# Ze-Yang/Context-Transformer

Hardware: AMD Instinct MI355X
Metric: images/sec fwd+NMS (higher is better)
Workload: dtype f32

## Files before the change

### context-transformer_amd/csrc/ct_conv.hip

```cpp
#include "ct_common.h"
#include "ct_conv_emit.h"
#include "ct_conv_launch.h"
#include "ct_device.h"
#include "ct_f16x2.h"
#include <algorithm>
#include <cmath>
#include <type_traits>
#include <cstdlib>

namespace {

using ctdet::f32x16;
using ctdet::i32x4;
using ctdet::kInvalidOff;
using ctdet::kMaxBufBytes;
using ctdet::make_rsrc;


struct ConvArgs {
    const float* in;
    const float* wpk;
    const float* scale;
    const float* shift;
    const float* res;
    const float* lo;
    float* out;
    unsigned in_bytes, w_bytes;
    int Cin, H, W, in_ctot, in_coff;
    int M, M_pad, nsteps;
    int stride, pad_h, pad_w, dil;
    int OW, OHW, Npix;
    int out_ctot, out_coff, res_ctot, res_coff;
    float res_scale;
    int relu;
    int nseg;
    ct_out_segment seg[3];
    int tiles_m, tiles_n;
    int transposed;
    int ksplit, steps_per_split;
    float* ws;
    unsigned* out_amax;
};

template <int KH, int KW, int CPB, int BM, int BN, int WAVES_M, int MINW>
__global__ __launch_bounds__(256, MINW) void conv_igemm_f32(const ConvArgs a)
{
    constexpr int KHW = KH * KW;
    constexpr int BK = CPB * KHW;
    constexpr int WAVES_N = 4 / WAVES_M;
    constexpr int WM = BM / WAVES_M, WN = BN / WAVES_N;
    constexpr int TM = WM / 32, TN = WN / 32;
    constexpr int RPP = 256 / BN;
    constexpr int NB = BK / RPP;
    constexpr int A_F4 = BK * BM / 4;
    constexpr int NA = (A_F4 + 255) / 256;
    static_assert(BK % 2 == 0 && BK % RPP == 0, "k-step must be even and divide into passes");
    static_assert(TM >= 1 && TN >= 1 && BN >= 64, "wave tile");

    extern __shared__ __attribute__((aligned(16))) float smem[];
    float* const As = smem;
    float* const Bs = smem + 2 * BK * BM;

    const int tid = threadIdx.x;
    const int lane = tid & 63;
    const int l31 = lane & 31;
    const int hsel = lane >> 5;
    const int wave = __builtin_amdgcn_readfirstlane(tid >> 6);
    const int wm0 = (wave % WAVES_M) * WM;
    const int wn0 = (wave / WAVES_M) * WN;

    int wg;
    {
        const int nwg = a.tiles_m * a.tiles_n;
        const int bid = blockIdx.x;
        const int xcd = bid & 7, local = bid >> 3;
        const int q = nwg >> 3, r = nwg & 7;
        wg = (xcd < r ? xcd * (q + 1) : r * (q + 1) + (xcd - r) * q) + local;
    }
    const int m0 = (wg % a.tiles_m) * BM;
    const int n0 = (wg / a.tiles_m) * BN;

    const __amdgpu_buffer_rsrc_t rin = make_rsrc(a.in, a.in_bytes);
    const __amdgpu_buffer_rsrc_t rw = make_rsrc(a.wpk, a.w_bytes);

    const int bp = tid % BN;
    const int rowgrp = __builtin_amdgcn_readfirstlane(tid / BN);
    const int HW = a.H * a.W;
    int img_base, oh_, ow_;
    bool pvalid;
    {
        const int P = n0 + bp;
        pvalid = P < a.Npix;
        const int Pc = pvalid ? P : 0;
        const int n = Pc / a.OHW;
        const int s = Pc - n * a.OHW;
        oh_ = s / a.OW;
        ow_ = s - oh_ * a.OW;
        img_base = (n * a.in_ctot + a.in_coff) * HW;
    }
    auto tap_offset = [&](int kh, int kw) -> int {
        int ih, iw;
        bool ok = pvalid;
        if (!a.transposed) {
            ih = oh_ * a.stride - a.pad_h + kh * a.dil;
            iw = ow_ * a.stride - a.pad_w + kw * a.dil;
        } else {
            const int th = oh_ + a.pad_h - kh * a.dil, tw = ow_ + a.pad_w - kw * a.dil;
            ih = th / a.stride;
            iw = tw / a.stride;
            ok = ok && th >= 0 && tw >= 0 && ih * a.stride == th && iw * a.stride == tw;
        }
        ok = ok && (unsigned)ih < (unsigned)a.H && (unsigned)iw < (unsigned)a.W;
        return ok ? img_base + ih * a.W + iw : -1;
    };

    int a_voff[NA];
    int a_lds[NA];
#pragma unroll
    for (int j = 0; j < NA; ++j) {
        int f = tid + 256 * j;
        if (f >= A_F4) f %= A_F4;
        const int arow = f / (BM / 4), ac4 = f % (BM / 4);
        const int col = m0 + ac4 * 4;
        a_voff[j] = (col < a.M_pad) ? (arow * a.M_pad + col) * 4 : kInvalidOff;
        a_lds[j] = arow * BM + ac4 * 4;
    }
    const int a_step_bytes = BK * a.M_pad * 4;

    int b_voff[NB];
    int b_chan[NB];
#pragma unroll
    for (int i = 0; i < NB; ++i) {
        const int r = rowgrp + RPP * i;
        const int c = r / KHW, tap = r - c * KHW;
        const int kh = tap / KW, kw = tap - kh * KW;
        const int off = tap_offset(kh, kw);
        b_voff[i] = off >= 0 ? off * 4 : kInvalidOff;
        b_chan[i] = c;
    }
    const int chan_bytes = HW * 4;

    i32x4 areg[NA];
    float breg[NB];

    auto load_elem = [&](int e, int step) {
        if (e < NA) {
            areg[e] = __builtin_amdgcn_raw_buffer_load_b128(rw, a_voff[e], step * a_step_bytes, 0);
        } else {
            const int i = e - NA;
            const int ci = step * CPB + b_chan[i];
            const int soff = (ci < a.Cin ? ci : 0) * chan_bytes;
            breg[i] = __builtin_bit_cast(float, __builtin_amdgcn_raw_buffer_load_b32(rin, b_voff[i], soff, 0));
        }
    };
    auto store_elem = [&](int e, int buf) {
        if (e < NA) {
            *reinterpret_cast<i32x4*>(As + buf * (BK * BM) + a_lds[e]) = areg[e];
        } else {
            const int i = e - NA;
            Bs[buf * (BK * BN) + (rowgrp + RPP * i) * BN + bp] = breg[i];
        }
    };
    auto load_tile = [&](int step) {
#pragma unroll
        for (int e = 0; e < NA + NB; ++e) load_elem(e, step);
    };
    auto store_tile = [&](int buf) {
#pragma unroll
        for (int e = 0; e < NA + NB; ++e) store_elem(e, buf);
    };

    f32x16 acc[TM][TN];
#pragma unroll
    for (int i = 0; i < TM; ++i)
#pragma unroll
        for (int j = 0; j < TN; ++j)
#pragma unroll
            for (int r = 0; r < 16; ++r) acc[i][j][r] = 0.f;

    constexpr int NKP = BK / 2;
    constexpr int NST = NA + NB;
    constexpr int NSLOT = NKP - 1;
    constexpr int WPS = (NST + NSLOT - 1) / NSLOT;

    const int s0 = blockIdx.y * a.steps_per_split;
    const int s1 = min(a.nsteps, s0 + a.steps_per_split);
    auto k_step = [&](int step, auto store_c, auto load_c) {
        constexpr bool STORE = decltype(store_c)::value, LOAD = decltype(load_c)::value;
        const int buf = (step - s0) & 1;
        const float* Ab = As + buf * (BK * BM) + hsel * BM + wm0 + l31;
        const float* Bb = Bs + buf * (BK * BN) + hsel * BN + wn0 + l31;
        float av[2][TM], bv[2][TN];
#pragma unroll
        for (int i = 0; i < TM; ++i) av[0][i] = Ab[i * 32];
#pragma unroll
        for (int j = 0; j < TN; ++j) bv[0][j] = Bb[j * 32];
#pragma unroll
        for (int kp = 0; kp < NKP; ++kp) {
            const int cur = kp & 1;
            if (kp + 1 < NKP) {
#pragma unroll
                for (int i = 0; i < TM; ++i) av[cur ^ 1][i] = Ab[(2 * kp + 2) * BM + i * 32];
#pragma unroll
                for (int j = 0; j < TN; ++j) bv[cur ^ 1][j] = Bb[(2 * kp + 2) * BN + j * 32];
            }
#pragma unroll
            for (int q = 0; q < WPS; ++q) {
                const int e = kp * WPS + q;
                if (e < NST) {
                    if (STORE) store_elem(e, buf ^ 1);
                    if (LOAD) load_elem(e, step + 2);
                }
            }
#pragma unroll
            for (int i = 0; i < TM; ++i)
#pragma unroll
                for (int j = 0; j < TN; ++j)
                    acc[i][j] = __builtin_amdgcn_mfma_f32_32x32x2f32(av[cur][i], bv[cur][j], acc[i][j], 0, 0, 0);
            __builtin_amdgcn_sched_barrier(0);
        }
        __syncthreads();
    };
    using T_ = std::true_type;
    using F_ = std::false_type;

    load_tile(s0);
    store_tile(0);
    if (s1 - s0 > 1) load_tile(s0 + 1);
    __syncthreads();
    int step = s0;
    for (; step + 2 < s1; ++step) k_step(step, T_{}, T_{});
    if (step + 1 < s1) { k_step(step, T_{}, F_{}); ++step; }
    k_step(step, F_{}, F_{});

    if (a.ksplit > 1) {
        float* const slab = a.ws + (size_t)blockIdx.y * a.M * a.Npix;
#pragma unroll
        for (int j = 0; j < TN; ++j) {
            const int P = n0 + wn0 + j * 32 + l31;
            if (P >= a.Npix) continue;
#pragma unroll
            for (int i = 0; i < TM; ++i)
#pragma unroll
                for (int r = 0; r < 16; ++r) {
                    const int co = m0 + wm0 + i * 32 + (r & 3) + 8 * (r >> 2) + 4 * hsel;
                    if (co < a.M) slab[(size_t)co * a.Npix + P] = acc[i][j][r];
                }
        }
        return;
    }

    float* const ev = smem;
    for (int i = tid; i < BM; i += 256) ctdet::stage_epilogue_vector<BM>(ev, a, m0, i);
    __syncthreads();
    const bool track = a.out_amax != nullptr;
#pragma unroll
    for (int j = 0; j < TN; ++j) {
        const int P = n0 + wn0 + j * 32 + l31;
        const bool live = P < a.Npix;
        const int n = live ? P / a.OHW : -1;
        float amax_run = 0.f;
        if (live) {
            const int s = P - n * a.OHW;
#pragma unroll
            for (int i = 0; i < TM; ++i) {
#pragma unroll
                for (int r = 0; r < 16; ++r) {
                    const int cl = wm0 + i * 32 + (r & 3) + 8 * (r >> 2) + 4 * hsel;
                    const int co = m0 + cl;
                    if (co >= a.M) continue;
                    float v = acc[i][j][r] * ev[cl] + ev[BM + cl];
                    if (a.res)
                        v = v * a.res_scale +
                            a.res[((size_t)n * a.res_ctot + a.res_coff + co) * a.OHW + s];
                    { const float fl = ev[2 * BM + cl]; v = v < fl ? fl : v; }
                    if (track) ctdet::h2::track_absmax(amax_run, v);
                    if (a.nseg == 0) {
                        a.out[((size_t)n * a.out_ctot + a.out_coff + co) * a.OHW + s] = v;
                    } else {
#pragma unroll
                        for (int g = 0; g < 3; ++g)
                            if (g < a.nseg && co >= a.seg[g].co_begin && co < a.seg[g].co_end)
                                a.seg[g].ptr[(size_t)n * a.seg[g].img_stride + a.seg[g].base +
                                             (size_t)s * a.seg[g].pix_stride + (co - a.seg[g].co_begin)] = v;
                    }
                }
            }
        }
        if (track) ctdet::h2::flush_absmax(a.out_amax, n, amax_run);
    }
}

template <int CIN, int PPT>
__global__ __launch_bounds__(256) void conv_valu3x3_f32(const ConvArgs a)
{
    typedef float f32x2 __attribute__((ext_vector_type(2)));
    constexpr int K = CIN * 9;
    const int HW = a.H * a.W;
    float x[PPT][K];
    float* op[PPT];
    bool live[PPT];
#pragma unroll
    for (int p = 0; p < PPT; ++p) {
        const int P = (blockIdx.x * PPT + p) * 256 + threadIdx.x;
        live[p] = P < a.Npix;
        const int Pc = live[p] ? P : 0;
        const int n = Pc / a.OHW, s = Pc - n * a.OHW;
        const int oh = s / a.OW, ow = s - oh * a.OW;
        const float* ip = a.in + ((size_t)n * a.in_ctot + a.in_coff) * HW;
#pragma unroll
        for (int kh = 0; kh < 3; ++kh) {
            const int ih = oh * a.stride - a.pad_h + kh * a.dil;
#pragma unroll
            for (int kw = 0; kw < 3; ++kw) {
                const int iw = ow * a.stride - a.pad_w + kw * a.dil;
                const bool ok = live[p] && (unsigned)ih < (unsigned)a.H && (unsigned)iw < (unsigned)a.W;
                const int off = ok ? ih * a.W + iw : 0;
#pragma unroll
                for (int ci = 0; ci < CIN; ++ci) {
                    const float v = ip[ci * HW + off];
                    x[p][ci * 9 + kh * 3 + kw] = ok ? v : 0.f;
                }
            }
        }
        op[p] = a.out + ((size_t)n * a.out_ctot + a.out_coff) * a.OHW + s;
    }
    typedef const __attribute__((address_space(4))) float cfloat;
    typedef const __attribute__((address_space(4))) f32x2 cf32x2;
    cfloat* const wk = (cfloat*)a.wpk;
    cfloat* const sc = (cfloat*)a.scale;
    cfloat* const sh = (cfloat*)a.shift;
    cfloat* const lo = (cfloat*)a.lo;
    float amax_run[PPT];
#pragma unroll
    for (int p = 0; p < PPT; ++p) amax_run[p] = 0.f;
    const bool track = a.out_amax != nullptr;
    for (int co0 = 0; co0 < a.M; co0 += 8) {
        f32x2 acc[PPT][4];
#pragma unroll
        for (int p = 0; p < PPT; ++p)
#pragma unroll
            for (int j = 0; j < 4; ++j) acc[p][j] = f32x2{0.f, 0.f};
        cfloat* wp = wk + co0;
        f32x2 wc[3][4], wn[3][4];
#pragma unroll
        for (int i = 0; i < 3; ++i)
#pragma unroll
            for (int j = 0; j < 4; ++j) wc[i][j] = ((cf32x2*)(wp + (size_t)i * a.M_pad))[j];
#pragma unroll
        for (int g = 0; g < K / 3; ++g) {
            {
                const f32x2 xx = f32x2{x[0][3 * g], x[0][3 * g]};
                acc[0][0] = __builtin_elementwise_fma(xx, wc[0][0], acc[0][0]);
            }
            __builtin_amdgcn_sched_barrier(0);
            if (g + 1 < K / 3) {
#pragma unroll
                for (int i = 0; i < 3; ++i)
#pragma unroll
                    for (int j = 0; j < 4; ++j) wn[i][j] = ((cf32x2*)(wp + (size_t)(3 * g + 3 + i) * a.M_pad))[j];
            }
            __builtin_amdgcn_sched_barrier(0);
#pragma unroll
            for (int p = 0; p < PPT; ++p)
#pragma unroll
                for (int i = 0; i < 3; ++i) {
                    const f32x2 xx = f32x2{x[p][3 * g + i], x[p][3 * g + i]};
#pragma unroll
                    for (int j = (p == 0 && i == 0 ? 1 : 0); j < 4; ++j)
                        acc[p][j] = __builtin_elementwise_fma(xx, wc[i][j], acc[p][j]);
                }
            __builtin_amdgcn_sched_barrier(0);
#pragma unroll
            for (int i = 0; i < 3; ++i)
#pragma unroll
                for (int j = 0; j < 4; ++j) wc[i][j] = wn[i][j];
        }
#pragma unroll
        for (int p = 0; p < PPT; ++p)
#pragma unroll
            for (int j = 0; j < 4; ++j) asm volatile("" : "+v"(acc[p][j]));
#pragma unroll
        for (int j = 0; j < 8; ++j) {
            const int co = co0 + j;
            const float scv = sc[co], shv = sh[co];
            const float lov = a.lo ? lo[co] : (a.relu ? 0.f : -INFINITY);
#pragma unroll
            for (int p = 0; p < PPT; ++p) {
                float v = (j & 1 ? acc[p][j >> 1].y : acc[p][j >> 1].x) * scv + shv;
                v = v < lov ? lov : v;
                if (live[p]) {
                    op[p][(size_t)co * a.OHW] = v;
                    if (track) ctdet::h2::track_absmax(amax_run[p], v);
                }
            }
        }
    }
    if (track) {
#pragma unroll
        for (int p = 0; p < PPT; ++p) {
            const int P = (blockIdx.x * PPT + p) * 256 + threadIdx.x;
            ctdet::h2::flush_absmax(a.out_amax, live[p] ? P / a.OHW : -1, amax_run[p]);
        }
    }
}

struct PackArgs {
    const float* w[6];
    int mbeg[7];
    int nparts, K, K_pad, M_pad;
    int dgrad, cin, khw;
    float* out;
};

__device__ __forceinline__ void pack_weights_body(const PackArgs& p, long first, long stride)
{
    const long total = (long)p.K_pad * p.M_pad;
    for (long idx = first; idx < total; idx += stride) {
        const int k = (int)(idx / p.M_pad), m = (int)(idx - (long)k * p.M_pad);
        float v = 0.f;
        if (!p.dgrad) {
            if (k < p.K) {
#pragma unroll
                for (int i = 0; i < 6; ++i)
                    if (i < p.nparts && m >= p.mbeg[i] && m < p.mbeg[i + 1])
                        v = p.w[i][(size_t)(m - p.mbeg[i]) * p.K + k];
            }
        } else if (k < p.K && m < p.cin) {
            const int co = k / p.khw, tap = k - co * p.khw;
#pragma unroll
            for (int i = 0; i < 6; ++i)
                if (i < p.nparts && co >= p.mbeg[i] && co < p.mbeg[i + 1])
                    v = p.w[i][((size_t)(co - p.mbeg[i]) * p.cin + m) * p.khw + tap];
        }
        p.out[idx] = v;
    }
}

__global__ void pack_weights_kernel(const PackArgs p)
{
    pack_weights_body(p, blockIdx.x * (long)blockDim.x + threadIdx.x, (long)gridDim.x * blockDim.x);
}

__global__ void pack_weights_batched_kernel(const PackArgs* __restrict__ items)
{
    const PackArgs p = items[blockIdx.y];
    pack_weights_body(p, blockIdx.x * (long)blockDim.x + threadIdx.x, (long)gridDim.x * blockDim.x);
}

__global__ void fold_epilogue_kernel(const float* gamma, const float* beta, const float* mean,
                                     const float* var, float eps, const float* bias, int n,
                                     float* scale, float* shift)
{
    const int i = blockIdx.x * blockDim.x + threadIdx.x;
    if (i >= n) return;
    if (gamma) {
        const float sc = gamma[i] / sqrtf(var[i] + eps);
        scale[i] = sc;
        shift[i] = beta[i] - mean[i] * sc;
    } else {
        scale[i] = 1.f;
        shift[i] = bias ? bias[i] : 0.f;
    }
}

struct TileCfg {
    int bm, bn, kmul;
    const char* name;
};
const TileCfg kCfgs[] = {
    {128, 128, 1, "128x128"}, {64, 128, 1, "64x128"}, {128, 64, 1, "128x64"}, {64, 64, 1, "64x64"},
    {32, 128, 1, "32x128"},   {160, 128, 1, "160x128"}, {128, 128, 2, "128x128k2"}, {96, 128, 1, "96x128"},
    {0, 256, 0, "valu"},
};
constexpr int kNumCfgs = sizeof(kCfgs) / sizeof(kCfgs[0]);
constexpr int kValuCfg = kNumCfgs - 1;

constexpr int cpb_for(int kh, int kw, int bn)
{
    return (kh == 3 && kw == 3) ? (bn == 128 ? 2 : 4)
         : (kh == 1 && kw == 1) ? 16
         : (kh * kw == 3)       ? (bn == 128 ? 6 : 4)
         : (kh == 4 && kw == 4) ? 1
                                : 0;
}

template <typename K>
hipError_t launch_one(K kernel, size_t smem, const ConvArgs& a, hipStream_t st)
{
    if (hipError_t e = ctdet::raise_lds_limit(reinterpret_cast<const void*>(kernel), smem)) return e;
    hipLaunchKernelGGL(kernel, dim3(a.tiles_m * a.tiles_n, a.ksplit > 1 ? a.ksplit : 1), dim3(256), smem, st, a);
    return hipGetLastError();
}

template <int KH, int KW>
hipError_t launch_geo(int cfg, const ConvArgs& a, hipStream_t st)
{
    switch (cfg) {
#define CT_CASE(idx, BM, BN, WMV, KMUL)                                                       \
    case idx: {                                                                               \
        constexpr int CPB = cpb_for(KH, KW, BN) * KMUL;                                       \
        constexpr size_t SMEM = (size_t)2 * CPB * KH * KW * (BM + BN) * sizeof(float);        \
                 \
        constexpr int MINW = (BM == 128 && BN == 128 && KMUL == 1) ? 4 : 1;                   \
        return launch_one(conv_igemm_f32<KH, KW, CPB, BM, BN, WMV, MINW>, SMEM, a, st);       \
    }
        CT_CASE(0, 128, 128, 2, 1)
        CT_CASE(1, 64, 128, 2, 1)
        CT_CASE(2, 128, 64, 2, 1)
        CT_CASE(3, 64, 64, 2, 1)
        CT_CASE(4, 32, 128, 1, 1)
        CT_CASE(5, 160, 128, 1, 1)
        CT_CASE(6, 128, 128, 2, 2)
        CT_CASE(7, 96, 128, 1, 1)
#undef CT_CASE
        default:
            return hipErrorInvalidValue;
    }
}

int pick_config(int M, long N)
{
    const int pad64 = (M + 63) / 64 * 64, pad128 = (M + 127) / 128 * 128;
    const int bm = M <= 32 ? 32 : (pad64 < pad128 ? 64 : 128);
    if (bm == 32) return 4;
    const long tm = (M + bm - 1) / bm;
    const long blocks128 = tm * ((N + 127) / 128);
    const bool small = blocks128 < 2 * 256;
    if (bm == 128) return small ? 2 : 0;
    return small ? 3 : 1;
}

}

extern "C" int ct_conv_kpad(int cin, int kh, int kw)
{
    if (cpb_for(kh, kw, 128) == 0) return -1;
    auto gcd = [](int a, int b) { while (b) { int t = a % b; a = b; b = t; } return a; };
    int l = 1;
    for (int i = 0; i < kNumCfgs; ++i) {
        if (i == kValuCfg) continue;
        const int c = cpb_for(kh, kw, kCfgs[i].bn) * kCfgs[i].kmul;
        l = l / gcd(l, c) * c;
    }
    return (cin + l - 1) / l * l * kh * kw;
}

extern "C" int ct_conv_mpad(int cout) { return (cout + 31) / 32 * 32; }

extern "C" int ct_conv_num_configs(void) { return kNumCfgs; }

extern "C" const char* ct_conv_config_name(int i)
{
    return (i >= 0 && i < kNumCfgs) ? kCfgs[i].name : "?";
}

static int pack_impl(const float* const* w, const int* cout, int nparts, int cin, int kh, int kw,
                     float* wpacked, int m_pad, int k_pad, int dgrad, ct_stream_t stream)
{
    CT_REQUIRE(nparts >= 1 && nparts <= 6, "ct_conv_pack_weights: nparts=%d (1..6)", nparts);
    PackArgs p{};
    int mtot = 0;
    for (int i = 0; i < nparts; ++i) {
        p.w[i] = w[i];
        p.mbeg[i] = mtot;
        mtot += cout[i];
    }
    p.mbeg[nparts] = mtot;
    for (int i = nparts + 1; i < 7; ++i) p.mbeg[i] = mtot;
    p.nparts = nparts;
    p.dgrad = dgrad;
    p.cin = cin;
    p.khw = kh * kw;
    if (!dgrad) {
        CT_REQUIRE(mtot <= m_pad, "ct_conv_pack_weights: sum(cout)=%d > m_pad=%d", mtot, m_pad);
        p.K = cin * kh * kw;
    } else {
        CT_REQUIRE(cin <= m_pad, "ct_conv_pack_weights_dgrad: cin=%d > m_pad=%d", cin, m_pad);
        p.K = mtot * kh * kw;
    }
    CT_REQUIRE(k_pad >= p.K, "ct_conv_pack_weights: k_pad=%d < K=%d", k_pad, p.K);
    p.K_pad = k_pad;
    p.M_pad = m_pad;
    p.out = wpacked;
    if (ctdet::pack_recording()) {
        ctdet::pack_record(0, &p, sizeof(p));
        return CT_OK;
    }
    const long total = (long)k_pad * m_pad;
    const int blocks = (int)std::min<long>((total + 255) / 256, 4096);
    hipLaunchKernelGGL(pack_weights_kernel, dim3(blocks), dim3(256), 0, ctdet::as_stream(stream), p);
    CT_LAUNCH_CHECK("pack_weights_kernel");
    return CT_OK;
}

size_t ctdet::pack_direct_item_bytes() { return sizeof(PackArgs); }

int ctdet::launch_pack_direct_batched(const void* items_dev, int n, hipStream_t st)
{
    if (n <= 0) return CT_OK;
    hipLaunchKernelGGL(pack_weights_batched_kernel, dim3(96, n), dim3(256), 0, st, (const PackArgs*)items_dev);
    CT_LAUNCH_CHECK("pack_weights_batched_kernel");
    return CT_OK;
}

extern "C" int ct_conv_pack_weights(const float* const* w, const int* cout, int nparts, int cin,
                                    int kh, int kw, float* wpacked, int m_pad, int k_pad,
                                    ct_stream_t stream)
{
    return pack_impl(w, cout, nparts, cin, kh, kw, wpacked, m_pad, k_pad, 0, stream);
}

extern "C" int ct_conv_pack_weights_dgrad(const float* const* w, const int* cout, int nparts, int cin,
                                          int kh, int kw, float* wpacked, int m_pad, int k_pad,
                                          ct_stream_t stream)
{
    return pack_impl(w, cout, nparts, cin, kh, kw, wpacked, m_pad, k_pad, 1, stream);
}

extern "C" int ct_conv_fold_epilogue(const float* gamma, const float* beta, const float* mean,
                                     const float* var, float eps, const float* bias, int n,
                                     int offset, float* scale, float* shift, ct_stream_t stream)
{
    CT_REQUIRE(n > 0 && offset >= 0, "ct_conv_fold_epilogue: n=%d offset=%d", n, offset);
    CT_REQUIRE(!gamma || (beta && mean && var), "ct_conv_fold_epilogue: BN needs beta/mean/var");
    hipLaunchKernelGGL(fold_epilogue_kernel, dim3((n + 255) / 256), dim3(256), 0,
                       ctdet::as_stream(stream), gamma, beta, mean, var, eps, bias, n,
                       scale + offset, shift + offset);
    CT_LAUNCH_CHECK("fold_epilogue_kernel");
    return CT_OK;
}

extern "C" int ct_conv2d_fwd(const ct_conv_desc* d, ct_stream_t stream)
{
    CT_REQUIRE(d != nullptr, "ct_conv2d_fwd: null descriptor");
    CT_REQUIRE(d->in && d->wpacked && d->scale && d->shift, "ct_conv2d_fwd: null tensor");
    CT_REQUIRE(d->batch > 0 && d->cin > 0 && d->cout > 0 && d->h > 0 && d->w > 0,
               "ct_conv2d_fwd: bad shape");
    CT_REQUIRE(d->stride >= 1 && d->dil >= 1, "ct_conv2d_fwd: stride/dilation");
    const char* const who = "ct_conv2d_fwd";
    if (int rc = ctdet::conv_check_sizes(d, who)) return rc;
    CT_REQUIRE(d->m_pad >= d->cout && d->m_pad % 4 == 0, "ct_conv2d_fwd: m_pad");
    const int kpad = ct_conv_kpad(d->cin, d->kh, d->kw);
    if (kpad < 0)
        return ctdet::fail(CT_ERR_UNSUPPORTED, "ct_conv2d_fwd: %dx%d filters not built", d->kh, d->kw);
    CT_REQUIRE(d->k_pad == kpad, "ct_conv2d_fwd: k_pad=%d, expected %d", d->k_pad, kpad);
    if (int rc = ctdet::conv_check_outputs(d, who)) return rc;
    CT_REQUIRE((long long)d->k_pad * d->m_pad * 4 < kMaxBufBytes, "ct_conv2d_fwd: weights too large");
    long long img_in_bytes;
    int max_chunk;
    if (int rc = ctdet::conv_check_image(d, who, &img_in_bytes, &max_chunk)) return rc;

    const bool valu_ok = d->kh == 3 && d->kw == 3 && d->cin == 3 && !d->transposed && d->nseg == 0 && !d->res &&
                         d->cout % 8 == 0 && d->batch <= max_chunk && (long long)d->batch * d->oh * d->ow < 0x7FFFFFFFLL;
    int cfg = d->config > 0 ? d->config - 1
            : valu_ok       ? kValuCfg
                            : pick_config(d->cout, (long)d->batch * d->oh * d->ow);
    CT_REQUIRE(cfg >= 0 && cfg < kNumCfgs, "ct_conv2d_fwd: config %d", d->config);
    if (cfg == kValuCfg) {
        if (!valu_ok)
            return ctdet::fail(CT_ERR_UNSUPPORTED, "ct_conv2d_fwd: config 'valu' is for 3x3 convolutions of 3 input channels "
                               "into a multiple of 8 output channels, NCHW output, no residual");
        ConvArgs a{};
        ctdet::conv_fill(a, d, 0, d->batch, img_in_bytes);
        a.wpk = d->wpacked;
        a.M_pad = d->m_pad;
        static const int ppt = getenv("CTDET_VALU_PPT") ? atoi(getenv("CTDET_VALU_PPT")) : 2;
        if (ppt == 1)
            hipLaunchKernelGGL((conv_valu3x3_f32<3, 1>), dim3((a.Npix + 255) / 256), dim3(256), 0, ctdet::as_stream(stream), a);
        else
            hipLaunchKernelGGL((conv_valu3x3_f32<3, 2>), dim3((a.Npix + 511) / 512), dim3(256), 0, ctdet::as_stream(stream), a);
        CT_LAUNCH_CHECK("conv_valu3x3_f32");
        return CT_OK;
    }
    const int bm = kCfgs[cfg].bm, bn = kCfgs[cfg].bn;
    const int cpb = cpb_for(d->kh, d->kw, bn) * kCfgs[cfg].kmul;

    for (int b0 = 0; b0 < d->batch; b0 += max_chunk) {
        const int nb = std::min(max_chunk, d->batch - b0);
        ConvArgs a{};
        ctdet::conv_fill(a, d, b0, nb, img_in_bytes);
        if (d->transposed) a.out_amax = nullptr;
        a.wpk = d->wpacked;
        a.w_bytes = (unsigned)((long long)d->k_pad * d->m_pad * 4);
        a.M_pad = d->m_pad;
        a.nsteps = (d->cin + cpb - 1) / cpb;
        a.tiles_m = (d->cout + bm - 1) / bm;
        a.tiles_n = (a.Npix + bn - 1) / bn;
        static const int target = getenv("CTDET_KSPLIT_TARGET") ? atoi(getenv("CTDET_KSPLIT_TARGET")) : 768;
        const ctdet::SplitK sk = ctdet::plan_splitk(d->ksplit, a.tiles_m * a.tiles_n, a.nsteps, (long long)d->cout * a.Npix,
                                                    d->ksplit_ws, d->ksplit_ws_floats, nb == d->batch, target);
        a.ksplit = sk.ksplit;
        a.steps_per_split = sk.steps_per_split;
        if (sk.ksplit > 1) a.ws = d->ksplit_ws;
        hipError_t e;
        hipStream_t st = ctdet::as_stream(stream);
        if (d->kh == 3 && d->kw == 3) e = launch_geo<3, 3>(cfg, a, st);
        else if (d->kh == 1 && d->kw == 1) e = launch_geo<1, 1>(cfg, a, st);
        else if (d->kh == 1 && d->kw == 3) e = launch_geo<1, 3>(cfg, a, st);
        else if (d->kh == 3 && d->kw == 1) e = launch_geo<3, 1>(cfg, a, st);
        else if (d->kh == 4 && d->kw == 4) e = launch_geo<4, 4>(cfg, a, st);
        else return ctdet::fail(CT_ERR_UNSUPPORTED, "ct_conv2d_fwd: %dx%d filters not built", d->kh, d->kw);
        if (e != hipSuccess)
            return ctdet::fail(CT_ERR_HIP, "conv_igemm_f32 launch failed: %s", hipGetErrorString(e));
        if (a.ksplit > 1) {
            const int total = a.M * a.Npix;
            hipLaunchKernelGGL(ctdet::conv_splitk_finish<ConvArgs>, dim3(std::min((total + 255) / 256, 2048)), dim3(256), 0, st, a);
            CT_LAUNCH_CHECK("conv_splitk_finish");
        }
    }
    return CT_OK;
}
```

### context-transformer_amd/csrc/ct_pool.hip

```cpp
#include "ct_common.h"
#include <algorithm>

namespace {

template <typename IDX>
__global__ __launch_bounds__(256) void maxpool2d_nchw(const float* __restrict__ in,
                                                      float* __restrict__ out, long planes, int H,
                                                      int W, int OH, int OW, int k, int stride, int pad)
{
    const IDX total = (IDX)(planes * OH * OW);
    for (IDX idx = (IDX)blockIdx.x * (IDX)blockDim.x + threadIdx.x; idx < total;
         idx += (IDX)gridDim.x * (IDX)blockDim.x) {
        const int ow = (int)(idx % OW);
        const IDX t = idx / OW;
        const int oh = (int)(t % OH);
        const IDX pl = t / OH;
        const int h0 = oh * stride - pad, w0 = ow * stride - pad;
        const int h1 = min(h0 + k, H), w1 = min(w0 + k, W);
        const float* p = in + (long)pl * H * W;
        float m = -INFINITY;
        for (int h = max(h0, 0); h < h1; ++h)
            for (int w = max(w0, 0); w < w1; ++w) m = fmaxf(m, p[h * W + w]);
        out[idx] = m;
    }
}

constexpr int P3_MAX_HW = 4096;
constexpr int P3_EPT = P3_MAX_HW / 256;

__global__ __launch_bounds__(256) void maxpool3x3s1_planes(const float* __restrict__ in, float* __restrict__ out, int planes,
                                                           int H, int W, int planes_per_wg)
{
    __shared__ float tile[2][P3_MAX_HW];
    const int HW = H * W, tid = threadIdx.x;
    int off[P3_EPT];
    unsigned mask[P3_EPT];
    const int n_e = (HW + 255) / 256;
#pragma unroll
    for (int j = 0; j < P3_EPT; ++j) {
        const int e = tid + 256 * j;
        off[j] = e;
        mask[j] = 0;
        if (j < n_e && e < HW) {
            const int h = e / W, w = e - h * W;
#pragma unroll
            for (int r = 0; r < 3; ++r)
#pragma unroll
                for (int c = 0; c < 3; ++c)
                    if ((unsigned)(h + r - 1) < (unsigned)H && (unsigned)(w + c - 1) < (unsigned)W) mask[j] |= 1u << (3 * r + c);
        }
    }
    const int p0 = blockIdx.x * planes_per_wg, p1 = min(planes, p0 + planes_per_wg);
    if (p0 >= p1) return;
    auto load = [&](int pl, int b) {
        const float* src = in + (size_t)pl * HW;
#pragma unroll
        for (int j = 0; j < P3_EPT; ++j)
            if (j < n_e && off[j] < HW) tile[b][off[j]] = src[off[j]];
    };
    load(p0, 0);
    __syncthreads();
    for (int pl = p0; pl < p1; ++pl) {
        const int b = (pl - p0) & 1;
        if (pl + 1 < p1) load(pl + 1, b ^ 1);
        float* dst = out + (size_t)pl * HW;
#pragma unroll
        for (int j = 0; j < P3_EPT; ++j) {
            if (j >= n_e || off[j] >= HW) continue;
            const float* c0 = &tile[b][off[j]];
            float m = -INFINITY;
#pragma unroll
            for (int r = 0; r < 3; ++r)
#pragma unroll
                for (int c = 0; c < 3; ++c)
                    if (mask[j] >> (3 * r + c) & 1u) m = fmaxf(m, c0[(r - 1) * W + (c - 1)]);
            dst[off[j]] = m;
        }
        __syncthreads();
    }
}

__global__ __launch_bounds__(256) void ctx_pool_nhwc(const float* __restrict__ in, long long in_img,
                                                     float* __restrict__ out, long long out_img,
                                                     int batch, int H, int W, int OH, int OW, int ch, int k)
{
    const long total = (long)batch * OH * OW * ch;
    for (long idx = blockIdx.x * (long)blockDim.x + threadIdx.x; idx < total;
         idx += (long)gridDim.x * blockDim.x) {
        const int c = (int)(idx % ch);
        long t = idx / ch;
        const int ow = (int)(t % OW);
        t /= OW;
        const int oh = (int)(t % OH);
        const int n = (int)(t / OH);
        const int h1 = min(oh * k + k, H), w1 = min(ow * k + k, W);
        const float* p = in + (long long)n * in_img;
        float m = -INFINITY;
        for (int h = oh * k; h < h1; ++h)
            for (int w = ow * k; w < w1; ++w) m = fmaxf(m, p[((long)h * W + w) * ch + c]);
        out[(long long)n * out_img + ((long)oh * OW + ow) * ch + c] = m;
    }
}

inline int grid_for(long total) { return (int)std::min<long>((total + 255) / 256, 256 * 16); }

}

extern "C" int ct_maxpool2d_fwd(const float* in, float* out, long planes, int h, int w, int oh, int ow,
                                int k, int stride, int pad, ct_stream_t stream)
{
    CT_REQUIRE(in && out && planes > 0 && h > 0 && w > 0 && oh > 0 && ow > 0, "ct_maxpool2d_fwd: bad shape");
    CT_REQUIRE(k >= 1 && stride >= 1 && pad >= 0 && pad < k, "ct_maxpool2d_fwd: k=%d stride=%d pad=%d", k, stride, pad);
    CT_REQUIRE((oh - 1) * stride - pad < h && (ow - 1) * stride - pad < w,
               "ct_maxpool2d_fwd: last window starts outside the input");
    if (k == 3 && stride == 1 && pad == 1 && oh == h && ow == w && h * w <= P3_MAX_HW && planes < 0x7FFFFFFFL) {
        const int ppw = (int)std::max<long>(2, (planes + 1023) / 1024);
        hipLaunchKernelGGL(maxpool3x3s1_planes, dim3((int)((planes + ppw - 1) / ppw)), dim3(256), 0, ctdet::as_stream(stream), in, out,
                           (int)planes, h, w, ppw);
        CT_LAUNCH_CHECK("maxpool3x3s1_planes");
        return CT_OK;
    }
    if (planes * oh * ow < 0x7FFFFFFFL)
        hipLaunchKernelGGL(maxpool2d_nchw<int>, dim3(grid_for(planes * oh * ow)), dim3(256), 0,
                           ctdet::as_stream(stream), in, out, planes, h, w, oh, ow, k, stride, pad);
    else
        hipLaunchKernelGGL(maxpool2d_nchw<long>, dim3(grid_for(planes * oh * ow)), dim3(256), 0,
                           ctdet::as_stream(stream), in, out, planes, h, w, oh, ow, k, stride, pad);
    CT_LAUNCH_CHECK("maxpool2d_nchw");
    return CT_OK;
}

extern "C" int ct_ctx_pool_fwd(const float* in, long long in_img_stride, float* out,
                               long long out_img_stride, int batch, int h, int w, int ch, int k,
                               ct_stream_t stream)
{
    CT_REQUIRE(in && out && batch > 0 && h > 0 && w > 0 && ch > 0 && k >= 1, "ct_ctx_pool_fwd: bad shape");
    const int oh = (h + k - 1) / k, ow = (w + k - 1) / k;
    hipLaunchKernelGGL(ctx_pool_nhwc, dim3(grid_for((long)batch * oh * ow * ch)), dim3(256), 0,
                       ctdet::as_stream(stream), in, in_img_stride, out, out_img_stride, batch, h, w,
                       oh, ow, ch, k);
    CT_LAUNCH_CHECK("ctx_pool_nhwc");
    return CT_OK;
}
```

Measured before the change: 4753.

## Vectorize 3x3 maxpool with packed plane groups and pack conv input registers

The 3x3 stride-1 maxpool kernel now packs several small planes into one shared-memory tile and loads and stores them with float4. It computes edge validity from per-element bit masks and builds the max from column maxima. It also uses a grid-stride loop with register-staged prefetch of the next group. Separately, the VALU 3x3 conv kernel stores its input patch as packed float pairs and broadcasts lanes by shuffle, aiming to get cheaper packed FMA operand handling. The maxpool rewrite adds indexing complexity and padding-boundary risks, and the conv change may shift register pressure.

```diff
diff --git a/context-transformer_amd/csrc/ct_conv.hip b/context-transformer_amd/csrc/ct_conv.hip
--- a/context-transformer_amd/csrc/ct_conv.hip
+++ b/context-transformer_amd/csrc/ct_conv.hip
@@ -297,7 +297,13 @@
     typedef float f32x2 __attribute__((ext_vector_type(2)));
     constexpr int K = CIN * 9;
     const int HW = a.H * a.W;
-    float x[PPT][K];
+    constexpr int NXP = (PPT * K + 1) / 2;
+    f32x2 xp[NXP];
+    xp[NXP - 1] = f32x2{0.f, 0.f};
+    auto xb = [&](int i) {
+        const f32x2 v = xp[i >> 1];
+        return i & 1 ? __builtin_shufflevector(v, v, 1, 1) : __builtin_shufflevector(v, v, 0, 0);
+    };
     float* op[PPT];
     bool live[PPT];
 #pragma unroll
@@ -319,7 +325,8 @@
 #pragma unroll
                 for (int ci = 0; ci < CIN; ++ci) {
                     const float v = ip[ci * HW + off];
-                    x[p][ci * 9 + kh * 3 + kw] = ok ? v : 0.f;
+                    const int i = p * K + ci * 9 + kh * 3 + kw;
+                    xp[i >> 1][i & 1] = ok ? v : 0.f;
                 }
             }
         }
@@ -336,6 +343,8 @@
     for (int p = 0; p < PPT; ++p) amax_run[p] = 0.f;
     const bool track = a.out_amax != nullptr;
     for (int co0 = 0; co0 < a.M; co0 += 8) {
+#pragma unroll
+        for (int i = 0; i < NXP; ++i) asm volatile("" : "+v"(xp[i]));
         f32x2 acc[PPT][4];
 #pragma unroll
         for (int p = 0; p < PPT; ++p)
@@ -350,8 +359,7 @@
 #pragma unroll
         for (int g = 0; g < K / 3; ++g) {
             {
-                const f32x2 xx = f32x2{x[0][3 * g], x[0][3 * g]};
-                acc[0][0] = __builtin_elementwise_fma(xx, wc[0][0], acc[0][0]);
+                acc[0][0] = __builtin_elementwise_fma(xb(3 * g), wc[0][0], acc[0][0]);
             }
             __builtin_amdgcn_sched_barrier(0);
             if (g + 1 < K / 3) {
@@ -365,7 +373,7 @@
             for (int p = 0; p < PPT; ++p)
 #pragma unroll
                 for (int i = 0; i < 3; ++i) {
-                    const f32x2 xx = f32x2{x[p][3 * g + i], x[p][3 * g + i]};
+                    const f32x2 xx = xb(p * K + 3 * g + i);
 #pragma unroll
                     for (int j = (p == 0 && i == 0 ? 1 : 0); j < 4; ++j)
                         acc[p][j] = __builtin_elementwise_fma(xx, wc[i][j], acc[p][j]);
diff --git a/context-transformer_amd/csrc/ct_pool.hip b/context-transformer_amd/csrc/ct_pool.hip
--- a/context-transformer_amd/csrc/ct_pool.hip
+++ b/context-transformer_amd/csrc/ct_pool.hip
@@ -26,56 +26,118 @@
 }
 
 constexpr int P3_MAX_HW = 4096;
-constexpr int P3_EPT = P3_MAX_HW / 256;
+constexpr int P3_PAD = 4;
+constexpr int P3_CPT = P3_MAX_HW / 4 / 256;
+
+__device__ __forceinline__ float p3_keep(float v, unsigned m, int bit)
+{
+    const unsigned all = (unsigned)((int)(m << (31 - bit)) >> 31);
+    return __builtin_bit_cast(float, (__builtin_bit_cast(unsigned, v) & all) | (0xFF800000u & ~all));
+}
 
 __global__ __launch_bounds__(256) void maxpool3x3s1_planes(const float* __restrict__ in, float* __restrict__ out, int planes,
-                                                           int H, int W, int planes_per_wg)
-{
-    __shared__ float tile[2][P3_MAX_HW];
+                                                           int H, int W, int G, int vec)
+{
+    __shared__ __attribute__((aligned(16))) float tile[2][P3_PAD + P3_MAX_HW + P3_PAD];
     const int HW = H * W, tid = threadIdx.x;
-    int off[P3_EPT];
-    unsigned mask[P3_EPT];
-    const int n_e = (HW + 255) / 256;
-#pragma unroll
-    for (int j = 0; j < P3_EPT; ++j) {
-        const int e = tid + 256 * j;
-        off[j] = e;
-        mask[j] = 0;
-        if (j < n_e && e < HW) {
-            const int h = e / W, w = e - h * W;
-#pragma unroll
-            for (int r = 0; r < 3; ++r)
-#pragma unroll
-                for (int c = 0; c < 3; ++c)
-                    if ((unsigned)(h + r - 1) < (unsigned)H && (unsigned)(w + c - 1) < (unsigned)W) mask[j] |= 1u << (3 * r + c);
-        }
-    }
-    const int p0 = blockIdx.x * planes_per_wg, p1 = min(planes, p0 + planes_per_wg);
-    if (p0 >= p1) return;
-    auto load = [&](int pl, int b) {
-        const float* src = in + (size_t)pl * HW;
-#pragma unroll
-        for (int j = 0; j < P3_EPT; ++j)
-            if (j < n_e && off[j] < HW) tile[b][off[j]] = src[off[j]];
+    const int cap = G * HW;
+    int up[P3_CPT], dn[P3_CPT];
+    unsigned mask[P3_CPT];
+#pragma unroll
+    for (int c = 0; c < P3_CPT; ++c) {
+        const int e = 4 * (tid + 256 * c);
+        unsigned m = 0;
+#pragma unroll
+        for (int k = 0; k < 4; ++k) {
+            if (e + k >= cap) continue;
+            const int p = (e + k) % HW, h = p / W, w = p - h * W;
+            m |= (unsigned)(h > 0) << (4 * k) | (unsigned)(h < H - 1) << (4 * k + 1) | (unsigned)(w > 0) << (4 * k + 2) |
+                 (unsigned)(w < W - 1) << (4 * k + 3);
+        }
+        mask[c] = m;
+        up[c] = m & 0x1111u ? W : 0;
+        dn[c] = m & 0x2222u ? W : 0;
+    }
+    const int ngroups = (planes + G - 1) / G;
+    int g = blockIdx.x;
+    if (g >= ngroups) return;
+    auto group_len = [&](int gi) { return min(G, planes - gi * G) * HW; };
+    float4 stage[P3_CPT];
+    auto fetch = [&](int gi) {
+        const float* src = in + (size_t)gi * cap;
+        const int ge = group_len(gi);
+        if (vec && !(ge & 3)) {
+#pragma unroll
+            for (int c = 0; c < P3_CPT; ++c) {
+                const int e = 4 * (tid + 256 * c);
+                if (e < ge) stage[c] = *(const float4*)(src + e);
+            }
+        } else {
+#pragma unroll
+            for (int c = 0; c < P3_CPT; ++c) {
+                const int e = 4 * (tid + 256 * c);
+                stage[c].x = e < ge ? src[e] : 0.f;
+                stage[c].y = e + 1 < ge ? src[e + 1] : 0.f;
+                stage[c].z = e + 2 < ge ? src[e + 2] : 0.f;
+                stage[c].w = e + 3 < ge ? src[e + 3] : 0.f;
+            }
+        }
     };
-    load(p0, 0);
+    auto stash = [&](int gi, int b) {
+        const int ge = group_len(gi);
+#pragma unroll
+        for (int c = 0; c < P3_CPT; ++c) {
+            const int e = 4 * (tid + 256 * c);
+            if (e < ge) *(float4*)&tile[b][P3_PAD + e] = stage[c];
+        }
+    };
+    fetch(g);
+    stash(g, 0);
     __syncthreads();
-    for (int pl = p0; pl < p1; ++pl) {
-        const int b = (pl - p0) & 1;
-        if (pl + 1 < p1) load(pl + 1, b ^ 1);
-        float* dst = out + (size_t)pl * HW;
-#pragma unroll
-        for (int j = 0; j < P3_EPT; ++j) {
-            if (j >= n_e || off[j] >= HW) continue;
-            const float* c0 = &tile[b][off[j]];
-            float m = -INFINITY;
-#pragma unroll
-            for (int r = 0; r < 3; ++r)
-#pragma unroll
-                for (int c = 0; c < 3; ++c)
-                    if (mask[j] >> (3 * r + c) & 1u) m = fmaxf(m, c0[(r - 1) * W + (c - 1)]);
-            dst[off[j]] = m;
-        }
+    for (int b = 0; g < ngroups; g += gridDim.x, b ^= 1) {
+        const int gn = g + gridDim.x;
+        if (gn < ngroups) fetch(gn);
+        const int ge = group_len(g);
+        float* dst = out + (size_t)g * cap;
+        float o[P3_CPT][4];
+#pragma unroll
+        for (int c = 0; c < P3_CPT; ++c) {
+            const int e = 4 * (tid + 256 * c);
+            if (e >= ge) continue;
+            const float* t = &tile[b][P3_PAD + e];
+            unsigned m = mask[c];
+            asm volatile("" : "+v"(m));
+            const float4 c4 = *(const float4*)t;
+            const float ctr[6] = {t[-1], c4.x, c4.y, c4.z, c4.w, t[4]};
+            float col[6];
+#pragma unroll
+            for (int i = 0; i < 6; ++i) {
+                const int k = i == 0 ? 0 : i == 5 ? 3 : i - 1;
+                const float a = t[i - 1 - up[c]], d = t[i - 1 + dn[c]];
+                col[i] = fmaxf(fmaxf(ctr[i], p3_keep(a, m, 4 * k)), p3_keep(d, m, 4 * k + 1));
+            }
+#pragma unroll
+            for (int k = 0; k < 4; ++k) {
+                const float l = p3_keep(col[k], m, 4 * k + 2), r = p3_keep(col[k + 2], m, 4 * k + 3);
+                o[c][k] = fmaxf(-INFINITY, fmaxf(fmaxf(col[k + 1], l), r));
+            }
+        }
+        if (vec && !(ge & 3)) {
+#pragma unroll
+            for (int c = 0; c < P3_CPT; ++c) {
+                const int e = 4 * (tid + 256 * c);
+                if (e < ge) *(float4*)(dst + e) = make_float4(o[c][0], o[c][1], o[c][2], o[c][3]);
+            }
+        } else {
+#pragma unroll
+            for (int c = 0; c < P3_CPT; ++c)
+#pragma unroll
+                for (int k = 0; k < 4; ++k) {
+                    const int e = 4 * (tid + 256 * c) + k;
+                    if (e < ge) dst[e] = o[c][k];
+                }
+        }
+        if (gn < ngroups) stash(gn, b ^ 1);
         __syncthreads();
     }
 }
@@ -114,9 +176,13 @@
     CT_REQUIRE((oh - 1) * stride - pad < h && (ow - 1) * stride - pad < w,
                "ct_maxpool2d_fwd: last window starts outside the input");
     if (k == 3 && stride == 1 && pad == 1 && oh == h && ow == w && h * w <= P3_MAX_HW && planes < 0x7FFFFFFFL) {
-        const int ppw = (int)std::max<long>(2, (planes + 1023) / 1024);
-        hipLaunchKernelGGL(maxpool3x3s1_planes, dim3((int)((planes + ppw - 1) / ppw)), dim3(256), 0, ctdet::as_stream(stream), in, out,
-                           (int)planes, h, w, ppw);
+        const int hw = h * w, step = hw % 4 == 0 ? 1 : hw % 2 == 0 ? 2 : 4;
+        const bool vec = step <= P3_MAX_HW / hw && ((uintptr_t)in | (uintptr_t)out) % 16 == 0;
+        const int q = vec ? step : 1;
+        const int G = (int)std::max<long>(q, std::min<long>(P3_MAX_HW / hw, planes / 256) / q * q);
+        const long ngroups = (planes + G - 1) / G;
+        hipLaunchKernelGGL(maxpool3x3s1_planes, dim3((int)std::min<long>(ngroups, 1024)), dim3(256), 0, ctdet::as_stream(stream), in, out,
+                           (int)planes, h, w, G, (int)vec);
         CT_LAUNCH_CHECK("maxpool3x3s1_planes");
         return CT_OK;
     }
```

After: 4799 (median of 6 runs). Within noise of the previous version (+1.0%).
